# wns349/tensorflow-yolo

Hardware: AMD Instinct MI355X
Metric: images/sec at 1/2/4/8 MI355X + post-NMS box-set match vs CPU ref (higher is better)
Workload: dtype f16; 1 GPU; v3-608-b32-fp16; network=v3, batch_per_gpu=32, global_batch=32, weights=seeded synthetic Darknet stream (random-init), streams=1

## Files before the change

### tensorflow-yolo_amd/csrc/stem.hip

```cpp
#include "conv_common.h"
#include <type_traits>

namespace yolo {

namespace {

typedef __attribute__((address_space(3))) void stem_lds_void;

__device__ __forceinline__ void stem_dma16(__amdgpu_buffer_rsrc_t rsrc, unsigned char *lds_dst, uint32_t voff) {
#if defined(__HIP_DEVICE_COMPILE__)
    __builtin_amdgcn_raw_ptr_buffer_load_lds(rsrc, (stem_lds_void *)lds_dst, 16, voff, 0, 0, 0);
#else
    (void)rsrc; (void)lds_dst; (void)voff;
#endif
}

__device__ __forceinline__ int stem_swz_w(int r) { return (0x78 >> (2 * ((r >> 2) & 3))) & 3; }
__device__ __forceinline__ int stem_swz_p(int r) { return (r >> 1) & 3; }

constexpr int TY = 8, TX = 16;
constexpr int P1Y = 2 * TY + 1;
constexpr int P1X = 2 * TX + 1;
constexpr int EVEN_COLS = (P1X + 1) / 2;
constexpr int ODD_COLS = P1X / 2;
constexpr int NEVEN = P1Y * EVEN_COLS;
constexpr int GEVEN = (NEVEN + 15) / 16;
constexpr int ODD0 = GEVEN * 16;
constexpr int NGRP = GEVEN + P1Y;
constexpr int INY = P1Y + 2, INX = P1X + 2;
constexpr int IN_PX = 36;
constexpr int IN_SKEW_PX = 32;
constexpr int IN_LD = IN_PX * 4 + 4;
constexpr int W2_BYTES = 9 * 64 * 64;
constexpr int P_BYTES = NGRP * 16 * 64;
constexpr int IN_BYTES = (INY * IN_LD * 2 + 15) / 16 * 16;
static_assert((W2_BYTES + P_BYTES + IN_BYTES) % 16 == 0 && (W2_BYTES + P_BYTES) % 16 == 0 && (IN_LD * 2) % 8 == 0,
              "LDS regions read with ds_read_b128 / b64 keep their alignment (a misaligned bias table cost 27 % of the kernel: SQ_LDS_UNALIGNED_STALL)");
static_assert(ODD0 + P1Y * ODD_COLS <= NGRP * 16 && 2 * (W2_BYTES + P_BYTES + IN_BYTES + (64 + 32) * 4) <= 160 * 1024, "patch rows / two workgroups per CU");
constexpr int BIAS_BYTES = (64 + 32) * 4;

}

template <bool U8>
__device__ __forceinline__ void stem_v3_body(const StemParams &p) {
    typedef _Float16 T;
    typedef typename std::conditional<U8, unsigned char, float>::type TIn;
    __shared__ __attribute__((aligned(16))) unsigned char smem[W2_BYTES + P_BYTES + IN_BYTES + BIAS_BYTES];
    unsigned char *const sW = smem;
    unsigned char *const sP = smem + W2_BYTES;
    T *const sIn = reinterpret_cast<T *>(smem + W2_BYTES + P_BYTES);
    float *const sBias = reinterpret_cast<float *>(smem + W2_BYTES + P_BYTES + IN_BYTES);

    const int tid = threadIdx.x;
    const int lane = tid & 63;
    const int wave = __builtin_amdgcn_readfirstlane(tid >> 6);
    const int fr = lane & 15, fq = lane >> 4;

    {
        const __amdgpu_buffer_rsrc_t rs_w = __builtin_amdgcn_make_buffer_rsrc(const_cast<void *>(p.w2), 0, p.w2_bytes, 0x00020000);
        const int lrow = lane >> 2;
        for (int i = wave; i < 36; i += 8) {
            const int tap = i >> 2, rg = i & 3;
            const int r = rg * 16 + lrow;
            const int co = 16 * ((r >> 2) & 3) + 4 * (r >> 4) + (r & 3);
            const uint32_t off = (uint32_t)co * p.wrow2 + (uint32_t)tap * 64 + (uint32_t)(((lane & 3) ^ stem_swz_w(lrow)) << 4);
            stem_dma16(rs_w, sW + i * 1024, off);
        }
    }
    uint4v a1[2][2];
    float4v bias1[2];
    {
#pragma unroll
        for (int t = 0; t < 2; ++t) {
            const int ch = 8 * (fr >> 2) + 4 * t + (fr & 3);
#pragma unroll
            for (int st = 0; st < 2; ++st) {
                T h[8];
#pragma unroll
                for (int j = 0; j < 8; ++j) {
                    const int kh = st == 0 ? (fq >> 1) : 2, pw = 2 * (fq & 1) + (j >> 2), c = j & 3;
                    const bool live = pw < 3 && c < 3 && (st == 0 || fq < 2);
                    const float w = p.w1[(live ? (kh * 3 + pw) * 3 + c : 0) * 32 + ch];
                    h[j] = live ? (T)w : (T)0.f;
                }
                __builtin_memcpy(&a1[t][st], h, 16);
            }
        }
        bias1[0] = *reinterpret_cast<const float4v *>(p.b1 + 8 * fq);
        bias1[1] = *reinterpret_cast<const float4v *>(p.b1 + 8 * fq + 4);
        if (tid < 64) sBias[tid] = p.b2[tid];
        else if (tid < 96 && p.w3) sBias[tid] = p.b3[tid - 64];
        for (int i = tid; i < INY * (IN_LD / 4); i += 512) *reinterpret_cast<unsigned long long *>(sIn + i * 4) = 0ull;
    }
    const int brow0 = (fq >> 1) * IN_LD;
    const int brow1 = (fq < 2 ? 2 : (fq >> 1)) * IN_LD;
    auto in_pix = [](int px) { return px * 4 + (px >= IN_SKEW_PX ? 4 : 0); };
    const int a_frag = fr * 64 + (((fq ^ stem_swz_w(fr)) & 3) << 4);
    uint4v a3[2][2];
    if (p.w3) {
#pragma unroll
        for (int t = 0; t < 2; ++t) {
            const int co = 8 * (fr >> 2) + 4 * t + (fr & 3);
#pragma unroll
            for (int ks = 0; ks < 2; ++ks)
                a3[t][ks] = *reinterpret_cast<const uint4v *>(reinterpret_cast<const unsigned char *>(p.w3) + co * 128 + (16 * fq + 8 * ks) * 2);
        }
    }

    constexpr int NIN = (INY + 3) / 4;
    typename std::conditional<U8, unsigned, float>::type in_r[NIN];
    const int in_col = tid & 127, in_row0 = tid >> 7;
    const bool in_col_ok = in_col < INX * 3;
    const int in_px = in_col / 3;
    T *const in_dst = sIn + in_row0 * IN_LD + in_pix(in_px) + (in_col - 3 * in_px);
    auto tile_origin = [&](int tile, int &n, int &oy0, int &ox0) {
        const uint32_t tyx = fdiv((uint32_t)tile, p.dtx);
        const int tx = (int)((uint32_t)tile - tyx * (uint32_t)p.tiles_x);
        n = (int)fdiv(tyx, p.dty);
        const int ty = (int)(tyx - (uint32_t)n * (uint32_t)p.tiles_y);
        oy0 = ty * TY; ox0 = tx * TX;
    };
    auto fetch_input = [&](int tile) {
        int n, oy0, ox0;
        tile_origin(tile, n, oy0, ox0);
        const TIn *img = reinterpret_cast<const TIn *>(p.in) + (long long)n * p.in_img_stride;
        const int gy0 = 2 * oy0 - 2 + in_row0, gx3 = (2 * ox0 - 2) * 3 + in_col;
        const bool xok = in_col_ok && (unsigned)gx3 < (unsigned)(3 * p.W);
        const int w3 = 3 * p.W;
#pragma unroll
        for (int it = 0; it < NIN; ++it) {
            const int gy = gy0 + 4 * it;
            const bool ok = xok && (unsigned)gy < (unsigned)p.H && (4 * it + in_row0 < INY);
            const TIn v = img[ok ? gy * w3 + gx3 : 0];
            in_r[it] = ok ? v : (TIn)0;
        }
    };

    int tile = blockIdx.x;
    fetch_input(tile);
    asm volatile("s_waitcnt vmcnt(0)" ::: "memory");
    __syncthreads();
    for (; tile < p.n_tiles; tile += gridDim.x) {
        int n, oy0, ox0;
        tile_origin(tile, n, oy0, ox0);
        const int y1_0 = 2 * oy0 - 1, x1_0 = 2 * ox0 - 1;
#pragma unroll
        for (int it = 0; it < NIN; ++it)
            if (in_col_ok && 4 * it + in_row0 < INY) {
                if constexpr (U8) in_dst[4 * it * IN_LD] = (T)u8_unit(in_r[it]);
                else in_dst[4 * it * IN_LD] = (T)in_r[it];
            }
        __syncthreads();
        if (tile + (int)gridDim.x < p.n_tiles) fetch_input(tile + gridDim.x);

        for (int g = wave; g < NGRP; g += 8) {
            const int rowP = g * 16 + fr;
            const bool live = g >= GEVEN || rowP < NEVEN;
            int py, px;
            if (g < GEVEN) {
                const int e = live ? rowP : NEVEN - 1;
                py = e / EVEN_COLS;
                px = 2 * (e - py * EVEN_COLS);
            } else {
                py = g - GEVEN;
                px = 2 * fr + 1;
            }
            const T *src = sIn + py * IN_LD;
            const int q0 = in_pix(px + 2 * (fq & 1)), q1 = in_pix(px + 2 * (fq & 1) + 1);
            typedef unsigned long long u64;
            const u64 b00 = *reinterpret_cast<const u64 *>(src + brow0 + q0), b01 = *reinterpret_cast<const u64 *>(src + brow0 + q1);
            const u64 b10 = *reinterpret_cast<const u64 *>(src + brow1 + q0), b11 = *reinterpret_cast<const u64 *>(src + brow1 + q1);
            uint4v b0, b1;
            b0.x = (unsigned)b00; b0.y = (unsigned)(b00 >> 32); b0.z = (unsigned)b01; b0.w = (unsigned)(b01 >> 32);
            b1.x = (unsigned)b10; b1.y = (unsigned)(b10 >> 32); b1.z = (unsigned)b11; b1.w = (unsigned)(b11 >> 32);
            float4v d0 = mma_chunk<T>(a1[0][0], b0, bias1[0]);
            float4v d1 = mma_chunk<T>(a1[1][0], b0, bias1[1]);
            d0 = mma_chunk<T>(a1[0][1], b1, d0);
            d1 = mma_chunk<T>(a1[1][1], b1, d1);
            const int gy = y1_0 + py, gx = x1_0 + px;
            const bool inside = (unsigned)gy < (unsigned)p.H && (unsigned)gx < (unsigned)p.W;
            T o[8];
#pragma unroll
            for (int j = 0; j < 4; ++j) {
                const float v0 = leaky01(d0[j]), v1 = leaky01(d1[j]);
                o[j] = (T)v0;
                o[4 + j] = (T)v1;
            }
            uint4v u;
            __builtin_memcpy(&u, o, 16);
            if (!inside) u = uint4v{0u, 0u, 0u, 0u};
            if (live) *reinterpret_cast<uint4v *>(sP + rowP * 64 + ((fq ^ stem_swz_p(rowP)) << 4)) = u;
        }
        __syncthreads();

        float4v acc[4];
#pragma unroll
        for (int a = 0; a < 4; ++a) acc[a] = *reinterpret_cast<const float4v *>(sBias + fq * 16 + 4 * a);
#pragma unroll
        for (int kh = 0; kh < 3; ++kh) {
            uint4v fb[3];
#pragma unroll
            for (int kw = 0; kw < 3; ++kw) {
                const int rowP = (kw & 1) ? ODD0 + (2 * wave + kh) * ODD_COLS + fr : (2 * wave + kh) * EVEN_COLS + fr + (kw >> 1);
                fb[kw] = *reinterpret_cast<const uint4v *>(sP + rowP * 64 + ((fq ^ stem_swz_p(rowP)) << 4));
            }
#pragma unroll
            for (int kw = 0; kw < 3; ++kw) {
                uint4v fa[4];
#pragma unroll
                for (int a = 0; a < 4; ++a) fa[a] = *reinterpret_cast<const uint4v *>(sW + (kh * 3 + kw) * 4096 + a * 1024 + a_frag);
#pragma unroll
                for (int a = 0; a < 4; ++a) acc[a] = mma_chunk<T>(fa[a], fb[kw], acc[a]);
            }
        }
        const int oy = oy0 + wave, ox = ox0 + fr;
        const bool valid = oy < p.Ho && ox < p.Wo;
        T o[16];
#pragma unroll
        for (int a = 0; a < 4; ++a)
#pragma unroll
            for (int j = 0; j < 4; ++j) {
                const float v = acc[a][j];
                o[4 * a + j] = (T)leaky01(v);
            }
        uint4v u0, u1;
        __builtin_memcpy(&u0, o, 16);
        __builtin_memcpy(&u1, o + 8, 16);
        const long long pix = (long long)oy * p.Wo + ox;
        if (valid) {
            T *op = reinterpret_cast<T *>(p.out) + (long long)n * p.out_img_stride + pix * p.out_ld + fq * 16;
            *reinterpret_cast<uint4v *>(op) = u0;
            *reinterpret_cast<uint4v *>(op + 8) = u1;
        }
        if (p.w3) {
            float4v d0 = mma_chunk<T>(a3[0][0], u0, *reinterpret_cast<const float4v *>(sBias + 64 + 8 * fq));
            float4v d1 = mma_chunk<T>(a3[1][0], u0, *reinterpret_cast<const float4v *>(sBias + 64 + 8 * fq + 4));
            d0 = mma_chunk<T>(a3[0][1], u1, d0);
            d1 = mma_chunk<T>(a3[1][1], u1, d1);
            T o3[8];
#pragma unroll
            for (int j = 0; j < 4; ++j) {
                const float v0 = d0[j], v1 = d1[j];
                o3[j] = (T)leaky01(v0);
                o3[4 + j] = (T)leaky01(v1);
            }
            uint4v u3;
            __builtin_memcpy(&u3, o3, 16);
            if (valid)
                *reinterpret_cast<uint4v *>(reinterpret_cast<T *>(p.out3) + (long long)n * p.out3_img_stride + pix * p.out3_ld + fq * 8) = u3;
        }
    }
}

__global__ void __launch_bounds__(512, 4) stem_v3_kernel(const StemParams p) { stem_v3_body<false>(p); }
__global__ void __launch_bounds__(512, 4) stem_v3_u8_kernel(const StemParams p) { stem_v3_body<true>(p); }

hipError_t launch_stem(const StemParams &p0, int batch, hipStream_t s, int max_grid, bool in_u8) {
    StemParams p = p0;
    if ((p.H & 1) || (p.W & 1) || p.Ho != p.H / 2 || p.Wo != p.W / 2) return hipErrorInvalidValue;
    p.tiles_x = (p.Wo + TX - 1) / TX;
    p.tiles_y = (p.Ho + TY - 1) / TY;
    p.dtx = make_fastdiv((uint32_t)p.tiles_x);
    p.dty = make_fastdiv((uint32_t)p.tiles_y);
    const long long tiles = (long long)batch * p.tiles_x * p.tiles_y;
    if (tiles <= 0 || tiles > 0x7fffffffLL) return hipErrorInvalidValue;
    p.n_tiles = (int)tiles;
    const unsigned grid = (unsigned)(tiles < max_grid ? tiles : max_grid);
    if (in_u8) hipLaunchKernelGGL(stem_v3_u8_kernel, dim3(grid), dim3(512), 0, s, p);
    else hipLaunchKernelGGL(stem_v3_kernel, dim3(grid), dim3(512), 0, s, p);
    return hipGetLastError();
}

}
```

Measured before the change: 6374 images/sec.

## Overlap stem input staging with layer-2 compute and specialize interior tiles

Restructures the persistent stem loop so the next tile's input is written to LDS right after layer 1 finishes, letting staging overlap the 3x3 conv phase instead of preceding layer 1. Interior tiles take a layer-1 path without per-pixel bounds checks, and edge masking of the input moves into staging. LDS read/write offsets for both layers and the output lane offsets are precomputed once per thread outside the tile loop. This trades extra registers (per-slot offsets, prefetch state) for less integer work and fewer serialized phases per tile, with some risk to occupancy under the 512x4 launch bound.

```diff
diff --git a/tensorflow-yolo_amd/csrc/stem.hip b/tensorflow-yolo_amd/csrc/stem.hip
--- a/tensorflow-yolo_amd/csrc/stem.hip
+++ b/tensorflow-yolo_amd/csrc/stem.hip
@@ -120,78 +120,137 @@
         const int ty = (int)(tyx - (uint32_t)n * (uint32_t)p.tiles_y);
         oy0 = ty * TY; ox0 = tx * TX;
     };
-    auto fetch_input = [&](int tile) {
-        int n, oy0, ox0;
-        tile_origin(tile, n, oy0, ox0);
+    const int w3 = 3 * p.W;
+    auto in_image = [&](int oy0, int ox0, bool (&ok)[NIN], int &idx0) {
+        const int gy0 = 2 * oy0 - 2 + in_row0, gx3 = (2 * ox0 - 2) * 3 + in_col;
+        const bool xok = in_col_ok && (unsigned)gx3 < (unsigned)w3;
+#pragma unroll
+        for (int it = 0; it < NIN; ++it) ok[it] = xok && (unsigned)(gy0 + 4 * it) < (unsigned)p.H && (4 * it + in_row0 < INY);
+        idx0 = gy0 * w3 + gx3;
+    };
+    auto fetch_input = [&](int n, int oy0, int ox0) {
         const TIn *img = reinterpret_cast<const TIn *>(p.in) + (long long)n * p.in_img_stride;
-        const int gy0 = 2 * oy0 - 2 + in_row0, gx3 = (2 * ox0 - 2) * 3 + in_col;
-        const bool xok = in_col_ok && (unsigned)gx3 < (unsigned)(3 * p.W);
-        const int w3 = 3 * p.W;
-#pragma unroll
-        for (int it = 0; it < NIN; ++it) {
-            const int gy = gy0 + 4 * it;
-            const bool ok = xok && (unsigned)gy < (unsigned)p.H && (4 * it + in_row0 < INY);
-            const TIn v = img[ok ? gy * w3 + gx3 : 0];
-            in_r[it] = ok ? v : (TIn)0;
-        }
-    };
-
-    int tile = blockIdx.x;
-    fetch_input(tile);
+        bool ok[NIN];
+        int idx0;
+        in_image(oy0, ox0, ok, idx0);
+#pragma unroll
+        for (int it = 0; it < NIN; ++it)
+            in_r[it] = img[ok[it] ? idx0 + 4 * it * w3 : 0];
+    };
+    auto stage_input = [&](int oy0, int ox0) {
+        const bool edge = oy0 == 0 || ox0 == 0 || 2 * oy0 + INY - 2 > p.H || 2 * ox0 + INX - 2 > p.W;
+        bool ok[NIN];
+        int idx0;
+        if (edge) in_image(oy0, ox0, ok, idx0);
+#pragma unroll
+        for (int it = 0; it < NIN; ++it)
+            if (in_col_ok && 4 * it + in_row0 < INY) {
+                T v;
+                if constexpr (U8) v = (T)u8_unit(in_r[it]);
+                else v = (T)in_r[it];
+                if (edge && !ok[it]) v = (T)0.f;
+                in_dst[4 * it * IN_LD] = v;
+            }
+    };
+
+    constexpr int NSLOT = (NGRP + 7) / 8;
+    static_assert(NEVEN > (GEVEN - 1) * 16 && ODD0 % 8 == 0 && ODD_COLS % 8 == 0, "only group GEVEN - 1 is partial; odd-column rows start at multiples of 8");
+    static_assert(8 * (NSLOT - 2) + 7 < NGRP, "every slot but the last holds a group for all 8 waves");
+    auto group_pos = [&](int g, int &py, int &px) {
+        if (g < GEVEN) {
+            const int e = g * 16 + fr < NEVEN ? g * 16 + fr : NEVEN - 1;
+            py = e / EVEN_COLS;
+            px = 2 * (e - py * EVEN_COLS);
+        } else {
+            py = g - GEVEN;
+            px = 2 * fr + 1;
+        }
+    };
+    int rd0[NSLOT], rd1[NSLOT];
+#pragma unroll
+    for (int k = 0; k < NSLOT; ++k) {
+        int py, px;
+        group_pos(wave + 8 * k < NGRP ? wave + 8 * k : NGRP - 1, py, px);
+        rd0[k] = (py * IN_LD + brow0 + in_pix(px + 2 * (fq & 1))) * 2;
+        rd1[k] = (py * IN_LD + brow0 + in_pix(px + 2 * (fq & 1) + 1)) * 2;
+    }
+    const int rd_row1 = (brow1 - brow0) * 2;
+    const int st_lane = fr * 64 + ((fq ^ stem_swz_p(fr)) << 4);
+    const bool live_last = fr < NEVEN - (GEVEN - 1) * 16;
+    int pf_even[3][2];
+#pragma unroll
+    for (int kh = 0; kh < 3; ++kh)
+#pragma unroll
+        for (int c = 0; c < 2; ++c) {
+            const int rowP = (2 * wave + kh) * EVEN_COLS + fr + c;
+            pf_even[kh][c] = rowP * 64 + ((fq ^ stem_swz_p(rowP)) << 4);
+        }
+    const int pf_odd = (ODD0 + 2 * wave * ODD_COLS) * 64 + st_lane;
+    const int out_lane = fr * p.out_ld + fq * 16, out3_lane = fr * p.out3_ld + fq * 8;
+    const unsigned char *const sInB = reinterpret_cast<const unsigned char *>(sIn);
+
+    auto layer1 = [&](auto edge_tag, int oy0, int ox0) {
+        constexpr bool EDGE = decltype(edge_tag)::value;
+#pragma unroll
+        for (int k = 0; k < NSLOT; ++k) {
+            const int g = wave + 8 * k;
+            if (k < NSLOT - 1 || g < NGRP) {
+                typedef unsigned long long u64;
+                const u64 b00 = *reinterpret_cast<const u64 *>(sInB + rd0[k]), b01 = *reinterpret_cast<const u64 *>(sInB + rd1[k]);
+                const u64 b10 = *reinterpret_cast<const u64 *>(sInB + rd0[k] + rd_row1), b11 = *reinterpret_cast<const u64 *>(sInB + rd1[k] + rd_row1);
+                uint4v b0, b1;
+                b0.x = (unsigned)b00; b0.y = (unsigned)(b00 >> 32); b0.z = (unsigned)b01; b0.w = (unsigned)(b01 >> 32);
+                b1.x = (unsigned)b10; b1.y = (unsigned)(b10 >> 32); b1.z = (unsigned)b11; b1.w = (unsigned)(b11 >> 32);
+                float4v d0 = mma_chunk<T>(a1[0][0], b0, bias1[0]);
+                float4v d1 = mma_chunk<T>(a1[1][0], b0, bias1[1]);
+                d0 = mma_chunk<T>(a1[0][1], b1, d0);
+                d1 = mma_chunk<T>(a1[1][1], b1, d1);
+                T o[8];
+#pragma unroll
+                for (int j = 0; j < 4; ++j) {
+                    const float v0 = leaky01(d0[j]), v1 = leaky01(d1[j]);
+                    o[j] = (T)v0;
+                    o[4 + j] = (T)v1;
+                }
+                uint4v u;
+                __builtin_memcpy(&u, o, 16);
+                if constexpr (EDGE) {
+                    int py, px;
+                    group_pos(g, py, px);
+                    const int gy = 2 * oy0 - 1 + py, gx = 2 * ox0 - 1 + px;
+                    const bool inside = (unsigned)gy < (unsigned)p.H && (unsigned)gx < (unsigned)p.W;
+                    if (!inside) u = uint4v{0u, 0u, 0u, 0u};
+                }
+                if ((g != GEVEN - 1) | live_last) *reinterpret_cast<uint4v *>(sP + st_lane + g * 1024) = u;
+            }
+        }
+    };
+
+    int tile = blockIdx.x, n, oy0, ox0, n1 = 0, oy1 = 0, ox1 = 0;
+    tile_origin(tile, n, oy0, ox0);
+    fetch_input(n, oy0, ox0);
     asm volatile("s_waitcnt vmcnt(0)" ::: "memory");
     __syncthreads();
-    for (; tile < p.n_tiles; tile += gridDim.x) {
-        int n, oy0, ox0;
-        tile_origin(tile, n, oy0, ox0);
-        const int y1_0 = 2 * oy0 - 1, x1_0 = 2 * ox0 - 1;
-#pragma unroll
-        for (int it = 0; it < NIN; ++it)
-            if (in_col_ok && 4 * it + in_row0 < INY) {
-                if constexpr (U8) in_dst[4 * it * IN_LD] = (T)u8_unit(in_r[it]);
-                else in_dst[4 * it * IN_LD] = (T)in_r[it];
-            }
+    stage_input(oy0, ox0);
+    if (tile + (int)gridDim.x < p.n_tiles) {
+        tile_origin(tile + gridDim.x, n1, oy1, ox1);
+        fetch_input(n1, oy1, ox1);
+    }
+    for (;;) {
         __syncthreads();
-        if (tile + (int)gridDim.x < p.n_tiles) fetch_input(tile + gridDim.x);
-
-        for (int g = wave; g < NGRP; g += 8) {
-            const int rowP = g * 16 + fr;
-            const bool live = g >= GEVEN || rowP < NEVEN;
-            int py, px;
-            if (g < GEVEN) {
-                const int e = live ? rowP : NEVEN - 1;
-                py = e / EVEN_COLS;
-                px = 2 * (e - py * EVEN_COLS);
-            } else {
-                py = g - GEVEN;
-                px = 2 * fr + 1;
-            }
-            const T *src = sIn + py * IN_LD;
-            const int q0 = in_pix(px + 2 * (fq & 1)), q1 = in_pix(px + 2 * (fq & 1) + 1);
-            typedef unsigned long long u64;
-            const u64 b00 = *reinterpret_cast<const u64 *>(src + brow0 + q0), b01 = *reinterpret_cast<const u64 *>(src + brow0 + q1);
-            const u64 b10 = *reinterpret_cast<const u64 *>(src + brow1 + q0), b11 = *reinterpret_cast<const u64 *>(src + brow1 + q1);
-            uint4v b0, b1;
-            b0.x = (unsigned)b00; b0.y = (unsigned)(b00 >> 32); b0.z = (unsigned)b01; b0.w = (unsigned)(b01 >> 32);
-            b1.x = (unsigned)b10; b1.y = (unsigned)(b10 >> 32); b1.z = (unsigned)b11; b1.w = (unsigned)(b11 >> 32);
-            float4v d0 = mma_chunk<T>(a1[0][0], b0, bias1[0]);
-            float4v d1 = mma_chunk<T>(a1[1][0], b0, bias1[1]);
-            d0 = mma_chunk<T>(a1[0][1], b1, d0);
-            d1 = mma_chunk<T>(a1[1][1], b1, d1);
-            const int gy = y1_0 + py, gx = x1_0 + px;
-            const bool inside = (unsigned)gy < (unsigned)p.H && (unsigned)gx < (unsigned)p.W;
-            T o[8];
-#pragma unroll
-            for (int j = 0; j < 4; ++j) {
-                const float v0 = leaky01(d0[j]), v1 = leaky01(d1[j]);
-                o[j] = (T)v0;
-                o[4 + j] = (T)v1;
-            }
-            uint4v u;
-            __builtin_memcpy(&u, o, 16);
-            if (!inside) u = uint4v{0u, 0u, 0u, 0u};
-            if (live) *reinterpret_cast<uint4v *>(sP + rowP * 64 + ((fq ^ stem_swz_p(rowP)) << 4)) = u;
-        }
+        if (oy0 == 0 || ox0 == 0 || 2 * oy0 + P1Y - 1 > p.H || 2 * ox0 + P1X - 1 > p.W) layer1(std::true_type(), oy0, ox0);
+        else layer1(std::false_type(), oy0, ox0);
         __syncthreads();
+        const int tile1 = tile + (int)gridDim.x;
+        const int n_cur = n, oy_cur = oy0, ox_cur = ox0;
+        if (tile1 < p.n_tiles) {
+            stage_input(oy1, ox1);
+            n = n1; oy0 = oy1; ox0 = ox1;
+            if (tile1 + (int)gridDim.x < p.n_tiles) {
+                tile_origin(tile1 + gridDim.x, n1, oy1, ox1);
+                fetch_input(n1, oy1, ox1);
+            }
+        }
 
         float4v acc[4];
 #pragma unroll
@@ -201,8 +260,7 @@
             uint4v fb[3];
 #pragma unroll
             for (int kw = 0; kw < 3; ++kw) {
-                const int rowP = (kw & 1) ? ODD0 + (2 * wave + kh) * ODD_COLS + fr : (2 * wave + kh) * EVEN_COLS + fr + (kw >> 1);
-                fb[kw] = *reinterpret_cast<const uint4v *>(sP + rowP * 64 + ((fq ^ stem_swz_p(rowP)) << 4));
+                fb[kw] = *reinterpret_cast<const uint4v *>(sP + ((kw & 1) ? pf_odd + kh * ODD_COLS * 64 : pf_even[kh][kw >> 1]));
             }
 #pragma unroll
             for (int kw = 0; kw < 3; ++kw) {
@@ -213,7 +271,7 @@
                 for (int a = 0; a < 4; ++a) acc[a] = mma_chunk<T>(fa[a], fb[kw], acc[a]);
             }
         }
-        const int oy = oy0 + wave, ox = ox0 + fr;
+        const int oy = oy_cur + wave, ox = ox_cur + fr;
         const bool valid = oy < p.Ho && ox < p.Wo;
         T o[16];
 #pragma unroll
@@ -226,9 +284,9 @@
         uint4v u0, u1;
         __builtin_memcpy(&u0, o, 16);
         __builtin_memcpy(&u1, o + 8, 16);
-        const long long pix = (long long)oy * p.Wo + ox;
+        const long long pix0 = (long long)oy * p.Wo + ox_cur;
         if (valid) {
-            T *op = reinterpret_cast<T *>(p.out) + (long long)n * p.out_img_stride + pix * p.out_ld + fq * 16;
+            T *op = reinterpret_cast<T *>(p.out) + ((long long)n_cur * p.out_img_stride + pix0 * p.out_ld) + out_lane;
             *reinterpret_cast<uint4v *>(op) = u0;
             *reinterpret_cast<uint4v *>(op + 8) = u1;
         }
@@ -247,8 +305,10 @@
             uint4v u3;
             __builtin_memcpy(&u3, o3, 16);
             if (valid)
-                *reinterpret_cast<uint4v *>(reinterpret_cast<T *>(p.out3) + (long long)n * p.out3_img_stride + pix * p.out3_ld + fq * 8) = u3;
-        }
+                *reinterpret_cast<uint4v *>(reinterpret_cast<T *>(p.out3) + ((long long)n_cur * p.out3_img_stride + pix0 * p.out3_ld) + out3_lane) = u3;
+        }
+        if (tile1 >= p.n_tiles) break;
+        tile = tile1;
     }
 }
 
```

Measured after the change: 6419 images/sec, median of 6. No clear change (+0.7%).
